# srv/pcl_feature_extraction

Hardware: AMD Instinct MI355X
Metric: Mpoints/s through NARF keypoint + FPFH descriptor on 1M-pt cloud (higher is better)
Workload: dtype f32; 1 GPU; configs[2] 1M-pt synthetic room, NARF(support 0.2) + normals(r 0.05) + FPFH(r 0.08) at the keypoints; image=640x480, parallelism=scan-per-gpu x1, descriptor_rows=83

## Files before the change

### pcl_feature_extraction_amd/csrc/pfx_grid.hip

```cpp
#include <algorithm>
#include <cstdlib>
#include <cstring>
#include <rocprim/rocprim.hpp>

#include "pfx_internal.h"

namespace pfx {
namespace {

__device__ __forceinline__ uint32_t f2ord(float f) {
  uint32_t u = __float_as_uint(f);
  return (u & 0x80000000u) ? ~u : (u | 0x80000000u);
}
__host__ __device__ __forceinline__ float ord2f(uint32_t u) {
  uint32_t b = (u & 0x80000000u) ? (u & 0x7fffffffu) : ~u;
  float f;
  memcpy(&f, &b, 4);
  return f;
}

constexpr int kBboxBlocks = 1024;
__global__ void __launch_bounds__(256) k_bbox(const float* __restrict__ x, const float* __restrict__ y,
                                              const float* __restrict__ z, int64_t n,
                                              uint32_t* __restrict__ mm) {
// ... 38 lines not shown
  uint32_t r[6] = {0xffffffffu, 0xffffffffu, 0xffffffffu, 0u, 0u, 0u};
  for (int b = t; b < nblocks; b += 256)
#pragma unroll
    for (int d = 0; d < 3; ++d) {
      r[d] = min(r[d], mm[b * 6 + d]);
      r[3 + d] = max(r[3 + d], mm[b * 6 + 3 + d]);
    }
#pragma unroll
  for (int d = 0; d < 6; ++d) s[d][t] = r[d];
  __syncthreads();
  for (int o = 128; o > 0; o >>= 1) {
    if (t < o)
#pragma unroll
      for (int d = 0; d < 3; ++d) {
        s[d][t] = min(s[d][t], s[d][t + o]);
        s[3 + d][t] = max(s[3 + d][t], s[3 + d][t + o]);
      }
    __syncthreads();
  }
  if (t < 6) mm[nblocks * 6 + t] = s[t][0];
}

__device__ __forceinline__ uint64_t lanemask_lt64() {
  const int lane = threadIdx.x & 63;
  return lane == 0 ? 0ull : (~0ull >> (64 - lane));
}

struct CellMap {
  double inv, ox, oy, oz, hx, hy, hz;
  int32_t nx, ny, nz;
};

__device__ __forceinline__ uint32_t point_key(const CellMap& m, float px, float py, float pz,
                                              int* __restrict__ oob) {
  uint32_t key = (uint32_t)((int64_t)m.nx * m.ny * m.nz);
  if (isfinite(px) && isfinite(py) && isfinite(pz)) {
    if (oob && ((double)px < m.ox || (double)py < m.oy || (double)pz < m.oz || (double)px > m.hx ||
                (double)py > m.hy || (double)pz > m.hz))
      atomicAdd(oob, 1);
    int64_t ix = (int64_t)floor(((double)px - m.ox) * m.inv);
    int64_t iy = (int64_t)floor(((double)py - m.oy) * m.inv);
    int64_t iz = (int64_t)floor(((double)pz - m.oz) * m.inv);
    ix = ix < 0 ? 0 : (ix >= m.nx ? m.nx - 1 : ix);
    iy = iy < 0 ? 0 : (iy >= m.ny ? m.ny - 1 : iy);
    iz = iz < 0 ? 0 : (iz >= m.nz ? m.nz - 1 : iz);
    key = (uint32_t)((ix * m.ny + iy) * m.nz + iz);
  }
  return key;
}

__global__ void __launch_bounds__(256) k_cell_keys(const float* __restrict__ x, const float* __restrict__ y,
                                                   const float* __restrict__ z, int64_t n, CellMap m,
                                                   uint32_t* __restrict__ keys, uint32_t* __restrict__ vals,
                                                   int* __restrict__ oob) {
  int64_t i = blockIdx.x * (int64_t)blockDim.x + threadIdx.x;
  if (i >= n) return;
  keys[i] = point_key(m, x[i], y[i], z[i], oob);
  vals[i] = (uint32_t)i;
}


constexpr int kCountBlock = 256;
constexpr int64_t kGridCountMaxPoints = int64_t(1) << 18;
constexpr int kAggRounds = 4;

__global__ void __launch_bounds__(256) k_count_zero(int32_t* __restrict__ p, int64_t m, int* __restrict__ oob) {
  for (int64_t i = blockIdx.x * (int64_t)blockDim.x + threadIdx.x; i < m; i += (int64_t)gridDim.x * blockDim.x)
    p[i] = 0;
  if (blockIdx.x == 0 && threadIdx.x == 0) *oob = 0;
}

__global__ void __launch_bounds__(kCountBlock) k_count_keys(const float* __restrict__ x, const float* __restrict__ y,
                                                            const float* __restrict__ z, int64_t n, CellMap m,
                                                            uint32_t* __restrict__ keys, uint32_t* __restrict__ rank,
                                                            int32_t* __restrict__ counts, int* __restrict__ oob) {
  const int64_t i = blockIdx.x * (int64_t)kCountBlock + threadIdx.x;
  const int lane = threadIdx.x & 63, wv = threadIdx.x >> 6;
  const uint32_t C = (uint32_t)((int64_t)m.nx * m.ny * m.nz);
  const bool live = i < n;
  uint32_t key = C;
  if (live) key = point_key(m, x[i], y[i], z[i], oob);
  const bool fin = live && key != C;
  uint64_t todo = __ballot(fin);
  int leader = lane, offs = 0, cnt = 1;
  for (int it = 0; it < kAggRounds && todo; ++it) {
    const int l = __builtin_ctzll(todo);
    const uint32_t k = (uint32_t)__shfl((int)key, l);
    const uint64_t same = __ballot(fin && key == k);
    if (fin && key == k) {
      leader = l;
      offs = __popcll(same & lanemask_lt64());
      cnt = __popcll(same);
    }
    todo &= ~same;
  }
  int base = 0;
  if (fin && lane == leader) base = atomicAdd(&counts[key], cnt);
  base = __shfl(base, leader);
  uint32_t r = (uint32_t)(base + offs);
  __shared__ int s_nf[kCountBlock / 64];
  const bool nf = live && !fin;
  const uint64_t bm = __ballot(nf);
  if (lane == 0) s_nf[wv] = __popcll(bm);
  __syncthreads();
  if (nf) {
    int before = __popcll(bm & lanemask_lt64());
    for (int w = 0; w < wv; ++w) before += s_nf[w];
    r = (uint32_t)before;
  }
// ... 37 lines not shown
    const int64_t last = s0 + 255 < n ? s0 + 255 : n - 1;
    const uint32_t k0 = skeys[s0], k1 = skeys[last];
    int64_t w0 = s0, w1 = s0;
    if (k0 < C) {
      w0 = cell_start[k0];
      w1 = cell_start[(k1 < C ? k1 : C - 1) + 1];
      w0 = w0 > s0 - kGridFatCap ? w0 : s0 - kGridFatCap;
      w1 = w1 < s0 + 256 + kGridFatCap ? w1 : s0 + 256 + kGridFatCap;
    }
    s_win[0] = w0;
    s_win[1] = w1;
  }
  __syncthreads();
  const int64_t w0 = s_win[0], w1 = s_win[1];
  for (int64_t t = w0 + threadIdx.x; t < w1; t += 256) s_idx[t - w0] = __float_as_uint(scr[t].w);
  __syncthreads();
  if (s >= n) return;
  const uint32_t key = skeys[s];
  const float4 v = scr[s];
  const uint32_t idx = __float_as_uint(v.w);
  int64_t d = s;
  if (key < C) {
    const int32_t start = cell_start[key], end = cell_start[key + 1];
    if (end - start > kGridFatCap) {
      if (s == start) atomicOr(oob, kGridFatBit);
      return;
    }
    const uint32_t* cell = s_idx + (start - w0);
    const int m = end - start;
    int before = 0;
    for (int t = 0; t < m; ++t) before += cell[t] < idx ? 1 : 0;
    d = (int64_t)start + before;
  }
  perm[d] = (int32_t)idx;
  sx[d] = v.x;
  sy[d] = v.y;
  sz[d] = v.z;
  sp[d] = make_float4(v.x, v.y, v.z, 0.0f);
}

__global__ void __launch_bounds__(256) k_fill_i32(int32_t* __restrict__ p, int64_t m, int32_t v) {
  for (int64_t i = blockIdx.x * (int64_t)blockDim.x + threadIdx.x; i < m; i += (int64_t)gridDim.x * blockDim.x)
    p[i] = v;
}

__global__ void __launch_bounds__(256) k_mark_starts(const uint32_t* __restrict__ skeys, int64_t n,
                                                     int32_t* __restrict__ cell_start) {
  const int64_t i = blockIdx.x * (int64_t)blockDim.x + threadIdx.x;
  if (i >= n) return;
  const uint32_t k = skeys[i];
  if (i == 0 || skeys[i - 1] != k) cell_start[k] = (int32_t)i;
}

__global__ void __launch_bounds__(256) k_gather_sorted(const float* __restrict__ x, const float* __restrict__ y,
                                                       const float* __restrict__ z, int64_t n,
                                                       const uint32_t* __restrict__ perm,
                                                       float* __restrict__ sx, float* __restrict__ sy,
                                                       float* __restrict__ sz, float4* __restrict__ sp) {
  int64_t i = blockIdx.x * (int64_t)blockDim.x + threadIdx.x;
  if (i >= n) return;
  uint32_t p = perm[i];
  const float a = x[p], b = y[p], c = z[p];
  sx[i] = a;
  sy[i] = b;
  sz[i] = c;
  sp[i] = make_float4(a, b, c, 0.0f);
}

__global__ void __launch_bounds__(256) k_fat_cells(const int32_t* __restrict__ cell_start, int64_t ncells,
                                                   int* __restrict__ flag) {
  const int64_t c = blockIdx.x * (int64_t)blockDim.x + threadIdx.x;
  if (c < ncells && cell_start[c + 1] - cell_start[c] > kGridFatCap) *flag = 1;
}

}

static bool bbox_dev(pfx_ctx* ctx, Grid& g, const float* d_x, const float* d_y, const float* d_z, int64_t n,
                     double lo[3], double hi[3]) {
  hipStream_t st = ctx->stream;
  uint32_t* mm = g.b_minmax.as<uint32_t>(6 * (kBboxBlocks + 1));
  const int blocks = (int)std::min<int64_t>(std::max<int64_t>(ceil_div(n, 1024), 1), kBboxBlocks);
  {
    TimeScope ts(ctx, "grid_bbox");
    k_bbox<<<blocks, 256, 0, st>>>(d_x, d_y, d_z, n, mm);
    k_bbox_reduce<<<1, 256, 0, st>>>(mm, blocks);
    check_launch("k_bbox");
  }
  uint32_t* h = ctx->readback<uint32_t>();
  PFX_HIP(hipMemcpyAsync(h, mm + 6 * blocks, sizeof(uint32_t) * 6, hipMemcpyDeviceToHost, st));
  ctx->sync_spin(st);
  uint32_t r[6];
  for (int d = 0; d < 6; ++d) r[d] = h[d];
  const bool any = r[0] != 0xffffffffu && r[3] != 0u;
  for (int d = 0; d < 3; ++d) {
    lo[d] = any ? ord2f(r[d]) : 0.0;
    hi[d] = any ? ord2f(r[3 + d]) : 0.0;
  }
  return any;
}

void points_bbox(pfx_ctx* ctx, Grid& g, const float* d_x, const float* d_y, const float* d_z, int64_t n,
                 double lo[3], double hi[3]) {
  bbox_dev(ctx, g, d_x, d_y, d_z, n, lo, hi);
}

void build_grid(pfx_ctx* ctx, Grid& g, const float* d_x, const float* d_y, const float* d_z,
                int64_t n, double radius, bool use_hint, bool fork_gather) {
  PFX_CHECK(n >= 0 && n < (int64_t(1) << 31), "point count must be in [0, 2^31)");
  PFX_CHECK(radius > 0.0, "radius must be > 0");
  ctx->join_side(ctx->stream);
  if (&g == &ctx->grid_b) {
    ctx->prep_x = nullptr;
    ctx->prep_n = -1;
    ctx->prep_qx = nullptr;
    ctx->prep_nq = -1;
  }
  hipStream_t st = ctx->stream;
  ++g.gen;
  g.n = n;
  g.ux = d_x; g.uy = d_y; g.uz = d_z;
  double lo[3] = {0, 0, 0}, hi[3] = {0, 0, 0};
  g.oob = nullptr;
  g.hint_user |= use_hint;
  if (use_hint && g.have_hint && n > 0) {
    for (int d = 0; d < 3; ++d) {
      lo[d] = g.hint_lo[d];
      hi[d] = g.hint_hi[d];
    }
    g.oob = g.b_oob.as<int>(1);
  } else if (n > 0) {
    bbox_dev(ctx, g, d_x, d_y, d_z, n, lo, hi);
    for (int d = 0; d < 3; ++d) {
      const double m = 0.1 * (hi[d] - lo[d]) + 2.0 * radius;
      g.hint_lo[d] = lo[d] - m;
      g.hint_hi[d] = hi[d] + m;
    }
    g.have_hint = true;
  }
  double cell = radius * (1.0 + 1e-6);
  const double max_cells = double(1 << 26);
  int64_t dims[3];
  for (int it = 0; it < 64; ++it) {
    for (int d = 0; d < 3; ++d) dims[d] = (int64_t)std::floor((hi[d] - lo[d]) / cell) + 1;
    double total = double(dims[0]) * double(dims[1]) * double(dims[2]);
    if (total <= max_cells) break;
    cell *= std::cbrt(total / max_cells) * 1.01;
  }
  g.cell = (float)cell;
  g.inv = (float)(1.0 / cell);
  g.ox = (float)lo[0]; g.oy = (float)lo[1]; g.oz = (float)lo[2];
  g.nx = (int32_t)dims[0]; g.ny = (int32_t)dims[1]; g.nz = (int32_t)dims[2];
  g.ncells = dims[0] * dims[1] * dims[2];
  const double inv = 1.0 / cell;
  g.inv = (float)inv;
  const int64_t C = g.ncells;

  const CellMap cm{inv, lo[0], lo[1], lo[2], hi[0], hi[1], hi[2], g.nx, g.ny, g.nz};
  g.dinv = inv;
  g.dox = lo[0]; g.doy = lo[1]; g.doz = lo[2];
  g.perm = g.b_perm.as<int32_t>(n + 1);
  g.sx = g.b_sx.as<float>(n + 1);
  g.sy = g.b_sy.as<float>(n + 1);
  g.sz = g.b_sz.as<float>(n + 1);
  g.sp = g.b_sp.as<float4>(n + 1);
  uint32_t* keys = g.b_keys.as<uint32_t>(n + 1);
  uint32_t* keys2 = g.b_keys2.as<uint32_t>(n + 1);
  uint32_t* vals = g.b_vals.as<uint32_t>(n + 1);
  g.skeys = keys2;

  if (g.oob && g.fat_pending) {
    PFX_HIP(hipEventSynchronize(g.fat_ev));
    g.fat_pending = false;
    g.fat = *g.h_fat != 0;
  }
  const char* mode = std::getenv("PFX_GRID_BUILD");
  const bool want_count = mode && std::strcmp(mode, "count") == 0
                              ? true
                              : (mode && std::strcmp(mode, "sort") == 0 ? false : n <= kGridCountMaxPoints);
  g.counted = g.oob != nullptr && n > 0 && want_count && !g.fat;
  ++ctx->stats[g.counted ? "grid_count_builds" : "grid_sort_builds"];
  if (g.oob && !g.counted) ++ctx->stats["grid_hinted_sort_builds"];
  if (g.counted) {
    const int64_t blocks = ceil_div(n, kCountBlock);
    const int64_t m = C + 1 + blocks;
    size_t scan_bytes = 0;
    PFX_HIP(rocprim::exclusive_scan(nullptr, scan_bytes, (int32_t*)nullptr, (int32_t*)nullptr, int32_t(0), (size_t)m,
                                    rocprim::plus<int32_t>(), st));
    void* tmp = g.b_tmp.get(scan_bytes + 16);
    g.cell_start = g.b_start.as<int32_t>(m + 1);
    float4* scr = g.b_scr.as<float4>(n + 1);
    TimeScope ts(ctx, "grid_build");
    k_count_zero<<<(unsigned)std::min<int64_t>(ceil_div(m, 256), 2048), 256, 0, st>>>(g.cell_start, m, g.oob);
    k_count_keys<<<(unsigned)blocks, kCountBlock, 0, st>>>(d_x, d_y, d_z, n, cm, keys, vals, g.cell_start, g.oob);
    check_launch("k_count_keys");
    PFX_HIP(rocprim::exclusive_scan(tmp, scan_bytes, g.cell_start, g.cell_start, int32_t(0), (size_t)m,
                                    rocprim::plus<int32_t>(), st));
    k_count_scatter<<<(unsigned)blocks, kCountBlock, 0, st>>>(d_x, d_y, d_z, n, (uint32_t)C, keys, vals, g.cell_start,
                                                              scr, keys2);
    k_count_order<<<(unsigned)ceil_div(n, 256), 256, 0, st>>>(scr, keys2, n, (uint32_t)C, g.cell_start, g.perm, g.sx,
                                                              g.sy, g.sz, g.sp, g.oob);
    check_launch("k_count_order");
    return;
  }

  using SortCfg = rocprim::radix_sort_config<rocprim::default_config, rocprim::default_config,
                                             rocprim::default_config, 0>;
  int bits = 1;
  while ((int64_t(1) << bits) <= C) ++bits;
  size_t sort_bytes = 0, scan_bytes = 0;
  PFX_HIP(rocprim::radix_sort_pairs<SortCfg>(nullptr, sort_bytes, (uint32_t*)nullptr, (uint32_t*)nullptr,
                                    (uint32_t*)nullptr, (uint32_t*)nullptr, (size_t)std::max<int64_t>(n, 1),
                                    0, bits, st));
  auto rev = rocprim::make_reverse_iterator(static_cast<int32_t*>(nullptr));
  PFX_HIP(rocprim::inclusive_scan(nullptr, scan_bytes, rev, rev, (size_t)(C + 1), rocprim::minimum<int32_t>(), st));
  void* tmp = g.b_tmp.get(std::max(sort_bytes, scan_bytes) + 16);
  g.cell_start = g.b_start.as<int32_t>(C + 2);
  {
    TimeScope ts(ctx, "grid_build");
    k_fill_i32<<<(unsigned)std::min<int64_t>(ceil_div(C + 2, 256), 2048), 256, 0, st>>>(g.cell_start, C + 2,
                                                                                       (int32_t)n);
    if (g.oob) k_fill_i32<<<1, 64, 0, st>>>(g.oob, 1, 0);
    if (n > 0) {
      k_cell_keys<<<(unsigned)ceil_div(n, 256), 256, 0, st>>>(d_x, d_y, d_z, n, cm, keys, vals, g.oob);
      check_launch("k_cell_keys");
      PFX_HIP(rocprim::radix_sort_pairs<SortCfg>(tmp, sort_bytes, keys, keys2, vals,
                                        reinterpret_cast<uint32_t*>(g.perm), (size_t)n, 0, bits, st));
      const bool forked = fork_gather && g.oob != nullptr;
      if (forked) ctx->fork_side(st);
      const auto gather = [&](hipStream_t s) {
        k_gather_sorted<<<(unsigned)ceil_div(n, 256), 256, 0, s>>>(d_x, d_y, d_z, n, reinterpret_cast<uint32_t*>(g.perm),
                                                                   g.sx, g.sy, g.sz, g.sp);
        check_launch("k_gather_sorted");
      };
      if (forked) gather(ctx->side);
      k_mark_starts<<<(unsigned)ceil_div(n, 256), 256, 0, st>>>(keys2, n, g.cell_start);
      auto r = rocprim::make_reverse_iterator(g.cell_start + C + 1);
      PFX_HIP(rocprim::inclusive_scan(tmp, scan_bytes, r, r, (size_t)(C + 1), rocprim::minimum<int32_t>(), st));
      if (!forked) gather(st);
    }
  }
  if (!g.oob && n > 0 && g.hint_user) {
    int* d_fat = g.b_fat.as<int>(1);
    if (!g.h_fat) PFX_HIP(hipHostMalloc((void**)&g.h_fat, 64, hipHostMallocDefault));
    if (!g.fat_ev) PFX_HIP(hipEventCreateWithFlags(&g.fat_ev, hipEventDisableTiming));
    if (g.fat_pending) PFX_HIP(hipEventSynchronize(g.fat_ev));
    k_fill_i32<<<1, 64, 0, st>>>(d_fat, 1, 0);
    k_fat_cells<<<(unsigned)ceil_div(C, 256), 256, 0, st>>>(g.cell_start, C, d_fat);
    check_launch("k_fat_cells");
    PFX_HIP(hipMemcpyAsync(g.h_fat, d_fat, sizeof(int), hipMemcpyDeviceToHost, st));
    PFX_HIP(hipEventRecord(g.fat_ev, st));
    g.fat_pending = true;
  }
}

}
```

### pcl_feature_extraction_amd/csrc/pfx_internal.h

```cpp
#pragma once
#include <hip/hip_runtime.h>
#include <stdint.h>
#include <cstdlib>

#include <map>
#include <stdexcept>
#include <string>
#include <vector>

#include "../../include/pfx.h"

namespace pfx {

struct Error : std::runtime_error {
  pfx_status code;
  Error(pfx_status c, const std::string& m) : std::runtime_error(m), code(c) {}
};

#define PFX_HIP(expr)                                                                   \
  do {                                                                                  \
    hipError_t _e = (expr);                                                             \
    if (_e != hipSuccess)                                                               \
      throw ::pfx::Error(PFX_ERR_DEVICE, std::string(#expr) + ": " + hipGetErrorString(_e)); \
  } while (0)

#define PFX_CHECK(cond, msg)                                                \
  do {                                                                      \
    if (!(cond)) throw ::pfx::Error(PFX_ERR_INVALID, std::string(msg));     \
  } while (0)

struct DevBuf {
  void* ptr = nullptr;
  size_t bytes = 0;
  void* get(size_t need) {
    if (need > bytes) {
      if (ptr) PFX_HIP(hipFree(ptr));
      size_t nb = need + need / 4 + 256;
      PFX_HIP(hipMalloc(&ptr, nb));
      bytes = nb;
    }
    return ptr;
  }
  template <class T> T* as(size_t count) { return static_cast<T*>(get(count * sizeof(T))); }
  void release() { if (ptr) (void)hipFree(ptr); ptr = nullptr; bytes = 0; }
};

struct KernelTimer {
  struct Pending { hipEvent_t a, b; std::string name; };
  bool enabled = false;
  bool stages_only = false;
  std::vector<Pending> pending;
  std::vector<hipEvent_t> pool;
  std::map<std::string, std::pair<double, int64_t> > acc;
  hipEvent_t take() {
    if (!pool.empty()) { hipEvent_t e = pool.back(); pool.pop_back(); return e; }
    hipEvent_t e;
    PFX_HIP(hipEventCreate(&e));
    return e;
  }
};

struct Grid {
  int64_t n = 0;
  float cell = 0.f, inv = 0.f, ox = 0.f, oy = 0.f, oz = 0.f;
  double dinv = 0.0, dox = 0.0, doy = 0.0, doz = 0.0;
  int32_t nx = 0, ny = 0, nz = 0;
  int64_t ncells = 0;
  float *sx = nullptr, *sy = nullptr, *sz = nullptr;
  float4* sp = nullptr;
  const float *ux = nullptr, *uy = nullptr, *uz = nullptr;
  int32_t* perm = nullptr;
  int32_t* cell_start = nullptr;
  const uint32_t* skeys = nullptr;
  DevBuf b_sx, b_sy, b_sz, b_sp, b_perm, b_start, b_keys, b_keys2, b_vals, b_tmp, b_minmax, b_oob, b_scr, b_fat;
  bool have_hint = false;
  double hint_lo[3] = {0, 0, 0}, hint_hi[3] = {0, 0, 0};
  int* oob = nullptr;
  mutable bool fat = false;
  int* h_fat = nullptr;
  hipEvent_t fat_ev = nullptr;
  bool fat_pending = false;
  bool hint_user = false;
  bool counted = false;
  uint64_t gen = 0;
  void release() {
    b_sx.release(); b_sy.release(); b_sz.release(); b_sp.release(); b_perm.release(); b_start.release();
    b_keys.release(); b_keys2.release(); b_vals.release(); b_tmp.release(); b_minmax.release(); b_oob.release();
    b_scr.release(); b_fat.release();
    if (fat_ev) { (void)hipEventSynchronize(fat_ev); (void)hipEventDestroy(fat_ev); fat_ev = nullptr; }
    if (h_fat) { (void)hipHostFree(h_fat); h_fat = nullptr; }
    fat_pending = false;
    have_hint = false;
    fat = false;
    oob = nullptr;
    ++gen;
  }
};

constexpr int kGridFatCap = 1024;
constexpr int kGridFatBit = 1 << 30;

struct GridView {
  const float *sx, *sy, *sz;
  const float4* sp;
  const float *ux, *uy, *uz;
  const int32_t* perm;
  const int32_t* cell_start;
  double inv, ox, oy, oz;
  int32_t nx, ny, nz;
};

enum ReportSlot {
  kRepFpfh, kRepPfh, kRepSpin, kRepIgrad, kRepRift, kRepSc, kRepLrf, kRepMoments, kRepPcurv, kReportSlots
};
constexpr int kReportWords = 16;
struct Reports {
  int* host = nullptr;
  bool pending[kReportSlots] = {};
  bool any() const {
    for (bool p : pending)
      if (p) return true;
    return false;
  }
};

struct NarfState;
struct NormalsState;
struct KeypointState;
struct IcpState;

}

struct pfx_ctx {
  int device = 0;
  hipStream_t own_stream = nullptr;
  hipStream_t stream = nullptr;
  bool on_own_stream = true;
  std::string last_error;
  bool shared_device = false;
  pfx::KernelTimer timer;
  std::map<std::string, int64_t> stats;
  pfx::Grid grid_a, grid_b;
  const float* prep_x = nullptr;
  int64_t prep_n = -1;
  double prep_r = 0.0;
  const float* prep_qx = nullptr;
  int64_t prep_nq = -1;
// ... 42 lines not shown
    PFX_HIP(hipEventRecord(fork_ev[1], side));
    PFX_HIP(hipStreamWaitEvent(st, fork_ev[1], 0));
  }
  void* host_rb = nullptr;
  template <class T> T* readback() {
    if (!host_rb) PFX_HIP(hipHostMalloc(&host_rb, 4096, hipHostMallocDefault));
    return static_cast<T*>(host_rb);
  }
  void* host_scratch = nullptr;
  size_t host_scratch_bytes = 0;
  void* pinned(size_t need) {
    if (need > host_scratch_bytes) {
      if (host_scratch) {
        PFX_HIP(hipStreamSynchronize(stream));
        PFX_HIP(hipHostFree(host_scratch));
      }
      host_scratch_bytes = need + need / 2 + 4096;
      PFX_HIP(hipHostMalloc(&host_scratch, host_scratch_bytes, hipHostMallocDefault));
    }
    return host_scratch;
  }
};

namespace pfx {

struct TimeScope {
  pfx_ctx* ctx;
  hipEvent_t a = nullptr, b = nullptr;
  std::string name;
  TimeScope(pfx_ctx* c, std::string n, bool stage = false) : ctx(c), name(std::move(n)) {
    if (ctx->timer.enabled && (stage || !ctx->timer.stages_only)) {
      a = ctx->timer.take();
      b = ctx->timer.take();
      PFX_HIP(hipEventRecord(a, ctx->stream));
    }
  }
  ~TimeScope() {
    if (a) {
      (void)hipEventRecord(b, ctx->stream);
      ctx->timer.pending.push_back(KernelTimer::Pending{a, b, name});
    }
  }
};

inline void check_launch(const char* what) {
  hipError_t e = hipGetLastError();
  if (e != hipSuccess)
    throw Error(PFX_ERR_DEVICE, std::string("launch ") + what + ": " + hipGetErrorString(e));
}

inline int64_t ceil_div(int64_t a, int64_t b) { return (a + b - 1) / b; }

void build_grid(pfx_ctx* ctx, Grid& g, const float* d_x, const float* d_y, const float* d_z,
                int64_t n, double radius, bool use_hint = false, bool fork_gather = false);
void points_bbox(pfx_ctx* ctx, Grid& g, const float* d_x, const float* d_y, const float* d_z, int64_t n,
                 double lo[3], double hi[3]);
inline void note_grid_word(pfx_ctx* ctx, const Grid& g, int word) {
  if (!(word & kGridFatBit)) return;
  g.fat = true;
  ++ctx->stats["grid_fat_fallbacks"];
}
inline GridView view(const Grid& g) {
  GridView v;
  v.sx = g.sx; v.sy = g.sy; v.sz = g.sz; v.sp = g.sp; v.perm = g.perm; v.cell_start = g.cell_start;
  v.ux = g.ux; v.uy = g.uy; v.uz = g.uz;
  v.inv = g.dinv; v.ox = g.dox; v.oy = g.doy; v.oz = g.doz; v.nx = g.nx; v.ny = g.ny; v.nz = g.nz;
  return v;
}

void normals_dev(pfx_ctx* ctx, const float* x, const float* y, const float* z, int64_t n,
                 double r, const float vp[3], float* nx, float* ny, float* nz, float* curv);
void normals_lists_dev(pfx_ctx* ctx, const float* x, const float* y, const float* z, int64_t n, double r,
                       float* nx, float* ny, float* nz, float* curv);
void normals_chains_dev(pfx_ctx* ctx, pfx_ctx* owner, const uint8_t* mask, int want, const float vp[3], float* nx,
                        float* ny, float* nz, float* curv);
void normals_release(pfx_ctx* ctx);
void normals_grid_launch_dev(pfx_ctx* ctx, const float* x, const float* y, const float* z, int64_t n, double r);
void normals_launch_dev(pfx_ctx* ctx, const float* x, const float* y, const float* z, int64_t n, double r,
                        const float vp[3], float* nx, float* ny, float* nz, float* curv);
bool normals_finish_dev(pfx_ctx* ctx);
void normals_prepare_dev(pfx_ctx* ctx, const float* x, const float* y, const float* z, int64_t n, double r);
void normals_subset_dev(pfx_ctx* ctx, const float* x, const float* y, const float* z, int64_t n, double r,
                        const uint8_t* mask, int want, const float vp[3], float* nx, float* ny, float* nz,
                        float* curv);
void normals_fast_dev(pfx_ctx* ctx, const float* x, const float* y, const float* z, int64_t n, double r,
                      const float vp[3], float* nx, float* ny, float* nz, float* curv);
double cloud_resolution_dev(pfx_ctx* ctx, const float* x, const float* y, const float* z, int64_t n);
int64_t iss_keypoints_dev(pfx_ctx* ctx, const float* x, const float* y, const float* z, int64_t n, double salient,
                          double non_max, int min_nb, double g21, double g32, int32_t* out, int64_t cap,
                          double* third_out);
void keypoints_release(pfx_ctx* ctx);
struct IcpResult {
  float T[16];
  double fitness;
  int converged, iterations, state;
};
void icp_dev(pfx_ctx* ctx, const float* sx, const float* sy, const float* sz, int64_t ns, const float* tx,
             const float* ty, const float* tz, int64_t nt, const pfx_icp_params& p, const float* guess,
             IcpResult& out, float* ax, float* ay, float* az);
void icp_release(pfx_ctx* ctx);
int64_t ransac_rejector(pfx_ctx* ctx, const float* sx, const float* sy, const float* sz, int64_t ns,
                        const float* tx, const float* ty, const float* tz, int64_t nt, const int32_t* query,
                        const int32_t* match, int64_t n, double threshold, int max_iterations, int32_t* keep_out,
                        float* T_out, int64_t* iters_out);
int64_t harris3d_dev(pfx_ctx* ctx, const float* x, const float* y, const float* z, int64_t n, double radius,
                     float threshold, int refine, int32_t* out, int64_t cap, float* resp_out, float* corners_out,
                     int64_t* n_corners, int32_t* corner_idx_out = nullptr);
// ... 87 lines not shown
```

### pcl_feature_extraction_amd/csrc/pfx_nblist.h

```cpp
#pragma once
#include "pfx_internal.h"
#include "pfx_neighbors.h"

namespace pfx {

constexpr uint32_t kEntryOffMask = 0x0fffffffu;
__host__ __device__ __forceinline__ int entry_run(uint32_t e) { return (int)(e >> 28); }
__host__ __device__ __forceinline__ uint32_t entry_off(uint32_t e) { return e & kEntryOffMask; }
constexpr uint8_t kLgCompact = 0x80;

__host__ __device__ __forceinline__ uint32_t widen_entry16(uint32_t e16) {
  return ((e16 >> 12) << 28) | (e16 & 0xfffu);
}
constexpr int kLaneMaxCompact = 2048;
__device__ __forceinline__ uint32_t list_entry(const uint32_t* list, int64_t off, int lgr, int m) {
  const int64_t i = off + ((int64_t)m << (lgr & 0x7f));
  return (lgr & kLgCompact) ? widen_entry16(reinterpret_cast<const uint16_t*>(list)[i]) : list[i];
}

struct NbLists {
  int64_t nq = 0;
  int64_t total = 0;
  int64_t long_total = 0;
  int64_t long_nq = 0;
// ... 14 lines not shown
constexpr int kLaneListLanes = 256;
constexpr int kLaneListTable = 9 * kLaneListLanes;

struct LaneList {
  int32_t p;
  int k;
  const uint32_t* lst;
  int lg;
  const int32_t* s_rt;
  int tid;

  __device__ __forceinline__ LaneList(const GridView& g, const NbLists& L, int64_t j, int32_t* table)
      : p(L.qpos[j]), s_rt(table), tid(threadIdx.x) {
    const uint32_t key = L.skeys[p];
#pragma unroll
    for (int r = 0; r < 9; ++r) {
      int32_t s, len;
      block_run(g, key, r, s, len);
      table[r * kLaneListLanes + tid] = s;
    }
    lst = L.list + L.off[j];
    lg = L.lg[j];
    k = L.cnt[j];
  }
  __device__ __forceinline__ uint32_t entry(int m) const { return lst[(int64_t)m << lg]; }
  __device__ __forceinline__ int32_t pos(int m) const {
    const uint32_t e = entry(m);
    return s_rt[entry_run(e) * kLaneListLanes + tid] + (int32_t)entry_off(e);
  }
  __device__ __forceinline__ int32_t idx(const GridView& g, int m) const { return g.perm[pos(m)]; }
};

constexpr int kLongList = 1024;

struct NormalsState {
  NbLists L;
  int64_t n = 0;
  const float *x = nullptr, *y = nullptr, *z = nullptr;
  double r = 0.0;
  bool ready = false;
  uint64_t grid_gen = 0;
  bool pending = false;
  bool nlong_zeroed = false;
  uint64_t grid_ahead_gen = 0;
  const float *grid_ahead_x = nullptr, *grid_ahead_y = nullptr, *grid_ahead_z = nullptr;
  int64_t grid_ahead_n = 0;
  double grid_ahead_r = 0.0;
  float vp[3] = {0.f, 0.f, 0.f};
  float *nx = nullptr, *ny = nullptr, *nz = nullptr, *curv = nullptr;
};

void build_lists(pfx_ctx* ctx, const Grid& g, const uint8_t* mask, double radius, bool sorted, NbLists& out,
                 const char* tag, bool defer = false, int want = 1, bool compact = false, bool gate = false);
bool build_lists_check(pfx_ctx* ctx, const Grid& g, NbLists& out, const char* tag);

}
```

### pcl_feature_extraction_amd/csrc/pfx_nblist.hip

```cpp
#include <cstdlib>
#include <cstring>
#include <rocprim/rocprim.hpp>

#include "pfx_nblist.h"
#include "pfx_neighbors.h"

namespace pfx {
namespace {

constexpr int kQ = 16;
typedef float pf2 __attribute__((ext_vector_type(2)));
constexpr int kArena = 16384;
constexpr int kArenaQuery = 16384;
constexpr int kTcapSmall = 384, kTcapSparse = 1280, kTcapDense = 8000;
constexpr int kCapQuery = 4096, kBucketsQuery = 1024;
constexpr int kCapMid8 = 8192, kBucketsMid8 = 1024;
constexpr int kCapMid = 16384, kBucketsMid = 2048;
#ifndef PFX_HUGE_BLOCKS
#define PFX_HUGE_BLOCKS 1024
#endif
constexpr int kCapHuge = 1 << 18, kBucketsHuge = 4096, kHugeBlocks = PFX_HUGE_BLOCKS;
#ifndef PFX_NT_QUERY
#define PFX_NT_QUERY 512
#endif
// ... 1572 lines not shown
  ListBuild(pfx_ctx* c, const Grid& grid, const char* t, double radius, bool sorted, bool compact_)
      : ctx(c), G(grid), tag(t), st(c->stream), n(grid.n), g(view(grid)), rr((float)(radius * radius)),
        isort(sorted ? 1 : 0), compact(compact_ ? 1 : 0), lb(buf("list")), hs(buf("scratch")) {
    qpos = buf("qpos").as<int32_t>(n);
    d_nq = buf("nq").as<int64_t>(1);
    flags = buf("flags").as<uint8_t>(n);
    seg = buf("seg").as<int32_t>(n);
    tiles = buf("tiles").as<int32_t>(n);
    d_ntiles = buf("ntiles").as<int64_t>(1);
    recs = buf("recs").as<int32_t>((size_t)2 * n * kRecInts);
    q4k = buf("single").as<int32_t>(n);
    qhuge = buf("huge").as<int32_t>(n);
    off = buf("off").as<int64_t>(n);
    cnt = buf("cnt").as<int32_t>(n);
    lgs = buf("lg").as<uint8_t>(n);
    counters = buf("counters").as<int>(kNCounters);
    wq = buf("wide").as<int32_t>((size_t)n);
    q16k = buf("mid").as<int32_t>(n);
    q8k = buf("mid8").as<int32_t>(n);
    qrec = buf("qrec").as<int32_t>((size_t)n * kRecInts);
    cursor = buf("cursor").as<unsigned long long>(4);
    PFX_HIP(rocprim::select(nullptr, t1, rocprim::counting_iterator<int32_t>(0), flags, qpos, d_nq, (size_t)n, st));
    PFX_HIP(rocprim::inclusive_scan(nullptr, t2, seg, seg, (size_t)n, rocprim::maximum<int32_t>(), st));
    PFX_HIP(rocprim::select(nullptr, t3, rocprim::counting_iterator<int32_t>(0), flags, tiles, d_ntiles, (size_t)n,
                            st));
    tmp = buf("tmp").get(std::max(t1, std::max(t2, t3)) + 16);
    tq_dev = static_cast<TierQ*>(buf("tierq").get(sizeof(TierQ)));
    if (!lb.ptr) {
      size_t words = 64 * (size_t)(n + 1);
      if (const char* e = std::getenv("PFX_LIST_WORDS")) words = std::max<size_t>(256, std::strtoull(e, nullptr, 10));
      lb.get(sizeof(uint32_t) * words);
    }
    const int heavy = (int)std::min<int64_t>(4, n >> 21);
    ch_small = 4;
    ch_sparse = std::max(2, heavy);
    ch_dense = std::max(1, heavy);
  }

  size_t list_words() const { return lb.bytes / sizeof(uint32_t); }
  ListOut list_out() const {
    return ListOut{off, cnt, lgs, static_cast<uint32_t*>(lb.ptr), cursor, list_words(), compact, qrec};
  }

  void setup(const uint8_t* mask, int want) {
    const unsigned nb = (unsigned)ceil_div(n, 256);
    const TierQ tq{{q4k, q8k, q16k, qhuge},
                   {counters + kWork4k, counters + kWork8k, counters + kWork16k, counters + kWorkHuge}};
    TimeScope ts(ctx, std::string(tag) + "_tiles");
    if (mask) {
      k_list_init<<<1, 256, 0, st>>>(nullptr, 0, nullptr, d_nq, counters, kNCounters, cursor, tq, tq_dev);
      k_mask_flags<<<nb, 256, 0, st>>>(G.perm, G.skeys, n, (uint64_t)G.ncells, mask, want, flags);
      PFX_HIP(rocprim::select(tmp, t1, rocprim::counting_iterator<int32_t>(0), flags, qpos, d_nq, (size_t)n, st));
    } else {
      k_list_init<<<nb, 256, 0, st>>>(qpos, n, G.cell_start + G.ncells, d_nq, counters, kNCounters, cursor, tq,
                                      tq_dev);
      const char* mode = std::getenv("PFX_LIST_SETUP");
      const bool cells = !(mode && std::strcmp(mode, "scan") == 0);
      ++ctx->stats[std::string(tag) + (cells ? "_setup_cells" : "_setup_scan")];
      if (cells) {
        k_tile_cells<<<(unsigned)ceil_div(n, kSlice), 256, 0, st>>>(g, G.skeys, G.ncells, recs, n, wq, counters);
        check_launch("nblist cell tiles");
        return;
      }
    }
    k_seg_marks<<<nb, 256, 0, st>>>(qpos, G.skeys, d_nq, seg);
    PFX_HIP(rocprim::inclusive_scan(tmp, t2, seg, seg, (size_t)n, rocprim::maximum<int32_t>(), st));
    k_tile_flags<<<nb, 256, 0, st>>>(seg, d_nq, flags, n);
    PFX_HIP(rocprim::select(tmp, t3, rocprim::counting_iterator<int32_t>(0), flags, tiles, d_ntiles, (size_t)n, st));
    k_tile_class<<<nb, 256, 0, st>>>(g, qpos, G.skeys, d_nq, tiles, d_ntiles, recs, n, wq, counters);
    check_launch("nblist tiles");
  }

  void reset_for_retry() {
    PFX_HIP(hipMemsetAsync(cursor, 0, 4 * sizeof(unsigned long long), st));
    PFX_HIP(hipMemsetAsync(counters + kRetryFirst, 0, (kNCounters - kRetryFirst) * sizeof(int), st));
  }

  template <int CAP, int NB, bool GLOBAL, int NT, int WPE>
  void launch_tier(unsigned grid, const int32_t* work, Counter count, Counter head, uint32_t* scratch,
                   const char* what) {
    const auto kern = k_nb_query<CAP, NB, GLOBAL, NT, WPE>;
    const size_t lds = GLOBAL ? 0 : sizeof(uint32_t) * 2 * CAP;
    if (lds) PFX_HIP(hipFuncSetAttribute((const void*)kern, hipFuncAttributeMaxDynamicSharedMemorySize, (int)lds));
    kern<<<grid, NT, lds, st>>>(g, work, counters + count, rr, (float)NB / rr, isort, list_out(),
                                GLOBAL ? nullptr : tq_dev, counters + kOverCap, scratch, counters + head);
    check_launch(what);
  }
  void launch_4k() {
    launch_tier<kCapQuery, kBucketsQuery, false, kNtQuery, PFX_Q_WPE>(kGrid4k, q4k, kWork4k, kHead4k, nullptr,
                                                                      "nblist 4k lists");
  }
  void launch_8k() {
    launch_tier<kCapMid8, kBucketsMid8, false, kNtMid8, kNtMid8 / 128>(kGrid8k, q8k, kWork8k, kHead8k, nullptr,
                                                                        "nblist 8k lists");
  }
  void launch_16k() {
    launch_tier<kCapMid, kBucketsMid, false, kNtMid, kNtMid / 256>(kGrid16k, q16k, kWork16k, kHead16k, nullptr,
                                                                    "nblist 16k lists");
  }
  unsigned huge_blocks() const { return (unsigned)std::min<size_t>(kGridHugeMax, hs.bytes / kHugeSlice); }
  void launch_huge() {
    launch_tier<kCapHuge, kBucketsHuge, true, kNtHuge, 4>(huge_blocks(), qhuge, kWorkHuge, kHeadHuge,
                                                          static_cast<uint32_t*>(hs.ptr), "nblist huge lists");
  }

  void launch_lists(int ran) {
    const ListOut lo = list_out();
    const float bscale = 256.0f / rr;
// ... 28 lines not shown
      TimeScope ts_query(ctx, std::string(tag) + "_lists_query");
      launch_4k();
      if (ran & kRan8k) launch_8k();
      if (ran & kRan16k) launch_16k();
      if (hs.ptr) launch_huge();
    }
    check_launch("nblist lists");
  }

  void defer_to_check(int ran, NbLists& out) {
    int64_t* d_nq_eff = buf("nq_eff").as<int64_t>(1);
    k_defer_gate<<<1, 64, 0, st>>>(counters, cursor, list_words(), hs.ptr ? 1 : 0, ran, G.oob, d_nq, d_nq_eff);
    check_launch("k_defer_gate");
    point(out);
    out.nq = n;
    out.nq_dev = d_nq_eff;
  }

  const ListsRb* read_back() { return pfx::read_back(ctx, counters, cursor, d_nq, nullptr); }
  int lack(const ListsRb* rb, int ran) const {
    return lists_lack(rb->cnt, rb->cur[0], list_words(), hs.ptr != nullptr, ran, rb->oob);
  }

  void catch_up(int lacking, int ran) {
    auto rewind = [&](Counter head, Counter count) {
      PFX_HIP(hipMemcpyAsync(counters + head, counters + count, sizeof(int), hipMemcpyDeviceToDevice, st));
    };
    if (ran & kRan16k) rewind(kHead16k, kWork16k);
    if (hs.ptr) rewind(kHeadHuge, kWorkHuge);
    if (lacking & kRan8k) launch_8k();
    launch_16k();
    if (hs.ptr) launch_huge();
  }

  void huge_alloc(int count) { hs.get(kHugeSlice * (size_t)std::min(kGridHugeMax, std::max(kCUs, count))); }

  void regrow(unsigned long long demand) {
    lb.release();
    lb.get(sizeof(uint32_t) * ((size_t)demand + kArenaTails + ((size_t)1 << 20)));
  }

  void point(NbLists& out) const {
    out.qpos = qpos;
    out.off = off;
    out.cnt = cnt;
    out.lg = lgs;
    out.list = static_cast<const uint32_t*>(lb.ptr);
    out.compact = compact != 0;
    out.list_cap = (int64_t)list_words();
    out.skeys = G.skeys;
  }
};

}

bool build_lists_check(pfx_ctx* ctx, const Grid& G, NbLists& out, const char* tag) {
  auto B = [&](const char* what) -> DevBuf& { return ctx->bufs[bname(tag, what)]; };
  const ListsRb* rb = read_back(ctx, B("counters").ptr, B("cursor").ptr, B("nq").ptr, G.oob);
  note_grid_word(ctx, G, rb->oob);
  const size_t words = B("list").bytes / sizeof(uint32_t);
  const int ran = (int)ctx->stats[std::string(tag) + "_ran_mid_tiers"];
  const int lacking = lists_lack(rb->cnt, rb->cur[0], words, B("scratch").ptr != nullptr, ran, rb->oob);
  if (lacking & (kLackGrid | kLackBuffer | kLackScratch)) return false;
  note_mid_tiers(ctx, tag, rb->cnt);
  if (lacking) return false;
  if (rb->cnt[kOverCap] > 0) throw_over_cap(tag, rb->cnt[kOverCap]);
  publish(ctx, tag, *rb, words, out);
  return true;
}

void build_lists(pfx_ctx* ctx, const Grid& G, const uint8_t* mask, double radius, bool sorted, NbLists& out,
                 const char* tag, bool defer, int want, bool compact, bool gate) {
  out = NbLists();
  if (G.n == 0) return;
  if (G.n >= (int64_t(1) << 28))
    throw Error(PFX_ERR_CAPACITY, std::string(tag) + ": neighbour lists support < 2^28 points");
  ListBuild b(ctx, G, tag, radius, sorted, compact);
  b.setup(mask, want);
  ctx->join_side(b.st);
  if (gate && ctx->lists_gate) {
    PFX_HIP(hipStreamWaitEvent(b.st, ctx->lists_gate, 0));
    ctx->lists_gate = nullptr;
  }
  for (int attempt = 0; attempt < 3; ++attempt) {
    if (attempt) b.reset_for_retry();
    int ran = attempt ? kRanAll : wanted_tiers(ctx, tag);
    ctx->stats[std::string(tag) + "_ran_mid_tiers"] = ran;
    b.launch_lists(ran);
    if (defer && attempt == 0) {
      b.defer_to_check(ran, out);
      return;
    }
    const ListsRb* rb = b.read_back();
    int lacking = b.lack(rb, ran);
    if (lacking & kRanWide) {
      note_mid_tiers(ctx, tag, rb->cnt);
      ++ctx->stats[std::string(tag) + "_wide_reruns"];
      continue;
    }
    if (lacking & (kRan8k | kRan16k)) {
      b.catch_up(lacking, ran);
      ran = kRanAll;
      rb = b.read_back();
      lacking = b.lack(rb, ran);
      ++ctx->stats[std::string(tag) + "_tier_catchups"];
    }
// ... 28 lines not shown
```

### pcl_feature_extraction_amd/csrc/pfx_normals.hip

```cpp
#include <cstring>
#include <algorithm>
#include <cstdio>
#include <cstdlib>
#include <mutex>

#include <rocprim/rocprim.hpp>

#include "pfx_nblist.h"
#include "pfx_neighbors.h"
#include "pfx_normal_math.h"

namespace pfx {
namespace {

constexpr int kBatch = 8;
#ifndef PFX_LANE_MAX
#define PFX_LANE_MAX (2 * kLongList)
#endif
constexpr int kLaneMax = PFX_LANE_MAX;
static_assert(kLaneMax >= kLaneMaxCompact, "lists up to kLaneMaxCompact must take the lane-per-query chains");

#ifndef PFX_LANE_DENSE_MUL
#define PFX_LANE_DENSE_MUL 2
#endif
// ... 705 lines not shown
    PFX_HIP(hipStreamSynchronize(st));
    ctx->stats["normals_long_lists"] = h[0];
    ctx->stats["normals_chain_wg_staged"] = h[1];
    ctx->stats["normals_chain_wg_table"] = h[2];
    ctx->stats["normals_chain_wg_lane"] = h[3];
    ctx->stats["normals_chain_wg_deferred"] = h[4];
  }
#ifdef PFX_SHOT_PROFILE
  {
    unsigned long long pr[16];
    PFX_HIP(hipStreamSynchronize(st));
    PFX_HIP(hipMemcpyFromSymbol(pr, HIP_SYMBOL(g_chain_prof), sizeof(pr)));
    for (int b = 0; b < 16; b += 8)
      fprintf(stderr, "chain%s: WGs %llu prologue %.0f cyc/WG | waves %llu chain %.0f cyc/wave, max k %.1f/wave, "
              "%.1f cyc/step, mean k %.1f/lane\n", b ? "_big" : "", pr[b + 4], pr[b + 0] / (double)(pr[b + 4] + !pr[b + 4]), pr[b + 3],
              pr[b + 1] / (double)(pr[b + 3] + !pr[b + 3]), pr[b + 2] / (double)(pr[b + 3] + !pr[b + 3]),
              pr[b + 1] / (double)(pr[b + 2] + !pr[b + 2]), pr[b + 5] / 64.0 / (double)(pr[b + 3] + !pr[b + 3]));
    const unsigned long long z[16] = {};
    PFX_HIP(hipMemcpyToSymbol(HIP_SYMBOL(g_chain_prof), z, sizeof(z)));
  }
#endif
}

namespace {

bool normals_speculative_lists(pfx_ctx* ctx, const float* x, const float* y, const float* z, int64_t n, double r,
                               float* nx, float* ny, float* nz, float* curv) {
  if (n == 0) return false;
  if (!ctx->normals) ctx->normals = new NormalsState();
  NormalsState& ns = *ctx->normals;
  ns.ready = false;
  ns.pending = false;
  ns.n = n;
  ns.x = x;
  ns.y = y;
  ns.z = z;
  ns.r = r;
  ns.L = NbLists();
  TimeScope phase(ctx, "normals_lists_phase", true);
  const bool ahead = ns.grid_ahead_gen != 0 && ns.grid_ahead_gen == ctx->grid_a.gen && ns.grid_ahead_x == x &&
                     ns.grid_ahead_y == y && ns.grid_ahead_z == z && ns.grid_ahead_n == n && ns.grid_ahead_r == r;
  ns.grid_ahead_gen = 0;
  struct SideJoin {
    pfx_ctx* ctx;
    ~SideJoin() {
      try {
        ctx->join_side(ctx->stream);
      } catch (...) {
      }
    }
  } side_join{ctx};
  const char* fork_env = std::getenv("PFX_GATHER_FORK");
  const bool fork_gather = !(fork_env && std::strcmp(fork_env, "0") == 0);
  if (!ahead) build_grid(ctx, ctx->grid_a, x, y, z, n, r, true, fork_gather);
  ctx->stats["normals_gather_forked"] += ctx->side_pending ? 1 : 0;
  int* n_long = ctx->buf("normals_nlong").as<int>(kNLong);
  k_nan_fill4<<<(unsigned)std::min<int64_t>(ceil_div(n, 256), 4096), 256, 0,
                ctx->side_pending ? ctx->side : ctx->stream>>>(nx, ny, nz, curv, n, n_long, kNLong);
  check_launch("k_nan_fill4");
  ns.nlong_zeroed = true;
  build_lists(ctx, ctx->grid_a, nullptr, r, true, ns.L, "normals", true, 1, true,
              true);
  return true;
}

bool normals_conclude(pfx_ctx* ctx, bool ok, const float* x, const float* y, const float* z, int64_t n, double r,
                      const float vp[3], float* nx, float* ny, float* nz, float* curv) {
  NormalsState& ns = *ctx->normals;
  ctx->grid_a.oob = nullptr;
  ctx->stats["normals_speculative_reruns"] += ok ? 0 : 1;
  if (ok) {
    ctx->stats["normals_neighbors"] = ns.L.total;
    ctx->stats["normals_long_neighbors"] = ns.L.long_total;
    ctx->stats["normals_long_queries"] = ns.L.long_nq;
    ctx->stats["normals_queries"] = ns.L.nq;
    ctx->normals_fork_hint = ns.L.long_nq * 8 <= ns.L.nq;
    return true;
  }
  normals_lists_dev(ctx, x, y, z, n, r, nx, ny, nz, curv);
  normals_chains_dev(ctx, ctx, nullptr, 0, vp, nx, ny, nz, curv);
  return false;
}
}

void normals_dev(pfx_ctx* ctx, const float* x, const float* y, const float* z, int64_t n, double r,
                 const float vp[3], float* nx, float* ny, float* nz, float* curv) {
  GateScope gate_scope(ctx);
  TimeScope total(ctx, "normals", true);
  PFX_CHECK(r > 0.0, "normals: radius must be > 0");
  PFX_CHECK(n >= 0, "normals: negative point count");
  if (normals_speculative_lists(ctx, x, y, z, n, r, nx, ny, nz, curv)) {
    NormalsState& ns = *ctx->normals;
    const bool ok = build_lists_check(ctx, ctx->grid_a, ns.L, "normals");
    ns.ready = true;
    if (ok) normals_chains_dev(ctx, ctx, nullptr, 0, vp, nx, ny, nz, curv);
    normals_conclude(ctx, ok, x, y, z, n, r, vp, nx, ny, nz, curv);
    return;
  }
  normals_lists_dev(ctx, x, y, z, n, r, nx, ny, nz, curv);
  if (n > 0) normals_chains_dev(ctx, ctx, nullptr, 0, vp, nx, ny, nz, curv);
}

void normals_launch_dev(pfx_ctx* ctx, const float* x, const float* y, const float* z, int64_t n, double r,
                        const float vp[3], float* nx, float* ny, float* nz, float* curv) {
  GateScope gate_scope(ctx);
  TimeScope total(ctx, "normals", true);
  PFX_CHECK(r > 0.0, "normals: radius must be > 0");
// ... 91 lines not shown
```

Baseline: 219.4 Mpoints/s.

## Replace fill+mark+min-scan cell starts with one fused kernel folding list init

Builds the grid's cell_start array in a single kernel. Slice blocks write each run boundary directly, and stripe blocks binary-search the sorted keys to fill the gaps between runs. This replaces the full-array fill, the mark-starts kernel and the reverse min-scan. The same kernel also performs the neighbor-list init work (qpos iota, counter and cursor reset, tier-queue blob copy), and the OOB word is double-buffered and zeroed inside k_cell_keys, which removes several small launches. The cost is considerably more complex code with packed 16-bit fields and extra coupling between grid build and list setup.

```diff
diff --git a/pcl_feature_extraction_amd/csrc/pfx_grid.hip b/pcl_feature_extraction_amd/csrc/pfx_grid.hip
--- a/pcl_feature_extraction_amd/csrc/pfx_grid.hip
+++ b/pcl_feature_extraction_amd/csrc/pfx_grid.hip
@@ -114,9 +114,10 @@
 __global__ void __launch_bounds__(256) k_cell_keys(const float* __restrict__ x, const float* __restrict__ y,
                                                    const float* __restrict__ z, int64_t n, CellMap m,
                                                    uint32_t* __restrict__ keys, uint32_t* __restrict__ vals,
-                                                   int* __restrict__ oob) {
+                                                   int* __restrict__ oob, int* __restrict__ oob_other) {
   int64_t i = blockIdx.x * (int64_t)blockDim.x + threadIdx.x;
   if (i >= n) return;
+  if (i == 0 && oob_other) *oob_other = 0;
   keys[i] = point_key(m, x[i], y[i], z[i], oob);
   vals[i] = (uint32_t)i;
 }
@@ -260,6 +261,101 @@
   if (i == 0 || skeys[i - 1] != k) cell_start[k] = (int32_t)i;
 }
 
+constexpr int kStartsSlice = 4096;
+constexpr int kStartsStripeBits = 11;
+__global__ void __launch_bounds__(256) k_cell_starts(const uint32_t* __restrict__ skeys, int64_t n, int64_t C,
+                                                     int32_t* __restrict__ cell_start, int nslices, GridTail tail) {
+  constexpr int slice = kStartsSlice;
+  constexpr int64_t T = int64_t(1) << kStartsStripeBits;
+  const int tid = threadIdx.x;
+  if ((int)blockIdx.x >= nslices) {
+    const int64_t S = (int64_t)(blockIdx.x - nslices) << kStartsStripeBits;
+    const int64_t E = S + T < C + 2 ? S + T : C + 2;
+    int64_t lo = 0, hi = n;
+    while (hi > lo) {
+      const int64_t step = (hi - lo + 255) / 256;
+      const int64_t at = lo + tid * step;
+      const int below = __syncthreads_count(at < hi && (int64_t)skeys[at] < E);
+      if (below == 0) {
+        hi = lo;
+      } else {
+        const int64_t h = lo + below * step;
+        lo = lo + (below - 1) * step + 1;
+        hi = h < hi ? h : hi;
+      }
+    }
+    const int64_t p = lo;
+    const int64_t k = p < n ? (int64_t)skeys[p] : C + 1;
+    const int64_t kp = p > 0 ? (int64_t)skeys[p - 1] : -1;
+    const int64_t c0 = kp + 1 > S ? kp + 1 : S;
+    const int64_t c1 = k - T < E - 1 ? k - T : E - 1;
+    for (int64_t c = c0 + tid; c <= c1; c += 256) cell_start[c] = (int32_t)p;
+    return;
+  }
+  __shared__ uint32_t s_key[kStartsSlice + 2];
+  __shared__ int32_t s_first[kStartsSlice + 1];
+  __shared__ uint32_t s_what[kStartsSlice + 1];
+  __shared__ int s_qn;
+  static_assert(kStartsStripeBits <= 16 && kStartsSlice <= 4096, "the packing of s_what");
+  const int64_t s0 = blockIdx.x * (int64_t)slice;
+  int m = (int)(n - s0 < slice ? n - s0 : slice);
+  {
+    uint32_t kr[kStartsSlice / 256];
+#pragma unroll
+    for (int i = 0; i < kStartsSlice / 256; ++i) kr[i] = tid + 256 * i < m ? skeys[s0 + tid + 256 * i] : 0u;
+#pragma unroll
+    for (int i = 0; i < kStartsSlice / 256; ++i)
+      if (tid + 256 * i < m) s_key[1 + tid + 256 * i] = kr[i];
+  }
+  if (tid == 0) {
+    s_key[0] = s0 > 0 ? skeys[s0 - 1] : 0xffffffffu;
+    s_qn = 0;
+    if (s0 + m == n) s_key[1 + m] = (uint32_t)(C + 1);
+  }
+  if (tail.qpos) {
+    for (int t = tid; t < m; t += 256) tail.qpos[s0 + t] = (int32_t)(s0 + t);
+    if (blockIdx.x == 0) {
+      if (tid < tail.ncounters) tail.counters[tid] = 0;
+      if (tid < 4) tail.cursor[tid] = 0ull;
+      if (tid == 0) {
+#pragma unroll
+        for (int w = 0; w < 8; ++w) tail.blob_dst[w] = tail.blob[w];
+      }
+    }
+  }
+  if (s0 + m == n) ++m;
+  __syncthreads();
+  for (int t = tid; t < m; t += 256) {
+    if (s_key[1 + t] == s_key[t]) continue;
+    const int64_t k = (int64_t)s_key[1 + t];
+    const int64_t kp = (s0 == 0 && t == 0) ? -1 : (int64_t)s_key[t];
+    const int64_t first = kp + 1 > k - (T - 1) ? kp + 1 : k - (T - 1);
+    if (tail.d_nq && k >= C && kp < C) *tail.d_nq = s0 + t;
+    if (k - first < 2) {
+      for (int64_t c = first; c <= k; ++c) cell_start[c] = (int32_t)(s0 + t);
+    } else {
+      const int e = atomicAdd(&s_qn, 1);
+      s_first[e] = (int32_t)first;
+      s_what[e] = ((uint32_t)t << 16) | (uint32_t)(k - first);
+    }
+  }
+  __syncthreads();
+  const int qn = s_qn, lane = tid & 63, wv = tid >> 6;
+  for (int base = 64 * wv; base < qn; base += 256) {
+    const int mine = base + lane < qn ? base + lane : qn - 1;
+    const int32_t f_l = s_first[mine];
+    const uint32_t w_l = s_what[mine];
+    const int ne = qn - base < 64 ? qn - base : 64;
+    for (int j = 0; j < ne; ++j) {
+      const int32_t f = __builtin_amdgcn_readlane(f_l, j);
+      const uint32_t w = (uint32_t)__builtin_amdgcn_readlane((int)w_l, j);
+      const int last = (int)(w & 0xffffu);
+      const int32_t v = (int32_t)(s0 + (w >> 16));
+      for (int c = lane; c <= last; c += 64) cell_start[(int64_t)f + c] = v;
+    }
+  }
+}
+
 __global__ void __launch_bounds__(256) k_gather_sorted(const float* __restrict__ x, const float* __restrict__ y,
                                                        const float* __restrict__ z, int64_t n,
                                                        const uint32_t* __restrict__ perm,
@@ -313,7 +409,7 @@
 }
 
 void build_grid(pfx_ctx* ctx, Grid& g, const float* d_x, const float* d_y, const float* d_z,
-                int64_t n, double radius, bool use_hint, bool fork_gather) {
+                int64_t n, double radius, bool use_hint, bool fork_gather, const GridTail* tail) {
   PFX_CHECK(n >= 0 && n < (int64_t(1) << 31), "point count must be in [0, 2^31)");
   PFX_CHECK(radius > 0.0, "radius must be > 0");
   ctx->join_side(ctx->stream);
@@ -325,6 +421,7 @@
   }
   hipStream_t st = ctx->stream;
   ++g.gen;
+  g.folded_init = nullptr;
   g.n = n;
   g.ux = d_x; g.uy = d_y; g.uz = d_z;
   double lo[3] = {0, 0, 0}, hi[3] = {0, 0, 0};
@@ -335,7 +432,13 @@
       lo[d] = g.hint_lo[d];
       hi[d] = g.hint_hi[d];
     }
-    g.oob = g.b_oob.as<int>(1);
+    const bool fresh = g.b_oob.ptr == nullptr;
+    int* words = g.b_oob.as<int>(2);
+    if (fresh) {
+      PFX_HIP(hipMemsetAsync(words, 0, 2 * sizeof(int), ctx->stream));
+      g.oob_next = 0;
+    }
+    g.oob = words + g.oob_next;
   } else if (n > 0) {
     bbox_dev(ctx, g, d_x, d_y, d_z, n, lo, hi);
     for (int d = 0; d < 3; ++d) {
@@ -388,6 +491,16 @@
   g.counted = g.oob != nullptr && n > 0 && want_count && !g.fat;
   ++ctx->stats[g.counted ? "grid_count_builds" : "grid_sort_builds"];
   if (g.oob && !g.counted) ++ctx->stats["grid_hinted_sort_builds"];
+  int* oob_other = nullptr;
+  if (g.oob) {
+    int* words = g.oob - g.oob_next;
+    if (g.counted) {
+      g.oob = words + (1 - g.oob_next);
+    } else {
+      oob_other = words + (1 - g.oob_next);
+      g.oob_next = 1 - g.oob_next;
+    }
+  }
   if (g.counted) {
     const int64_t blocks = ceil_div(n, kCountBlock);
     const int64_t m = C + 1 + blocks;
@@ -425,11 +538,15 @@
   g.cell_start = g.b_start.as<int32_t>(C + 2);
   {
     TimeScope ts(ctx, "grid_build");
-    k_fill_i32<<<(unsigned)std::min<int64_t>(ceil_div(C + 2, 256), 2048), 256, 0, st>>>(g.cell_start, C + 2,
-                                                                                       (int32_t)n);
-    if (g.oob) k_fill_i32<<<1, 64, 0, st>>>(g.oob, 1, 0);
+    const char* starts_env = std::getenv("PFX_CELL_STARTS");
+    const bool scan_starts = n == 0 || (starts_env && std::strcmp(starts_env, "scan") == 0);
+    ctx->stats["grid_starts_scan"] += scan_starts ? 1 : 0;
+    ctx->stats["grid_starts_fill"] += scan_starts ? 0 : 1;
+    if (scan_starts)
+      k_fill_i32<<<(unsigned)std::min<int64_t>(ceil_div(C + 2, 256), 2048), 256, 0, st>>>(g.cell_start, C + 2,
+                                                                                         (int32_t)n);
     if (n > 0) {
-      k_cell_keys<<<(unsigned)ceil_div(n, 256), 256, 0, st>>>(d_x, d_y, d_z, n, cm, keys, vals, g.oob);
+      k_cell_keys<<<(unsigned)ceil_div(n, 256), 256, 0, st>>>(d_x, d_y, d_z, n, cm, keys, vals, g.oob, oob_other);
       check_launch("k_cell_keys");
       PFX_HIP(rocprim::radix_sort_pairs<SortCfg>(tmp, sort_bytes, keys, keys2, vals,
                                         reinterpret_cast<uint32_t*>(g.perm), (size_t)n, 0, bits, st));
@@ -441,9 +558,19 @@
         check_launch("k_gather_sorted");
       };
       if (forked) gather(ctx->side);
-      k_mark_starts<<<(unsigned)ceil_div(n, 256), 256, 0, st>>>(keys2, n, g.cell_start);
-      auto r = rocprim::make_reverse_iterator(g.cell_start + C + 1);
-      PFX_HIP(rocprim::inclusive_scan(tmp, scan_bytes, r, r, (size_t)(C + 1), rocprim::minimum<int32_t>(), st));
+      if (scan_starts) {
+        k_mark_starts<<<(unsigned)ceil_div(n, 256), 256, 0, st>>>(keys2, n, g.cell_start);
+        auto r = rocprim::make_reverse_iterator(g.cell_start + C + 1);
+        PFX_HIP(rocprim::inclusive_scan(tmp, scan_bytes, r, r, (size_t)(C + 1), rocprim::minimum<int32_t>(), st));
+      } else {
+        const int nslices = (int)ceil_div(n, kStartsSlice);
+        const int nstripes = (int)ceil_div(C + 2, int64_t(1) << kStartsStripeBits);
+        const bool fold = tail && tail->qpos && g.oob != nullptr;
+        k_cell_starts<<<(unsigned)(nslices + nstripes), 256, 0, st>>>(keys2, n, C, g.cell_start, nslices,
+                                                                      fold ? *tail : GridTail());
+        if (fold) g.folded_init = tail->qpos;
+        check_launch("k_cell_starts");
+      }
       if (!forked) gather(st);
     }
   }
diff --git a/pcl_feature_extraction_amd/csrc/pfx_internal.h b/pcl_feature_extraction_amd/csrc/pfx_internal.h
--- a/pcl_feature_extraction_amd/csrc/pfx_internal.h
+++ b/pcl_feature_extraction_amd/csrc/pfx_internal.h
@@ -58,6 +58,16 @@
     PFX_HIP(hipEventCreate(&e));
     return e;
   }
+};
+
+struct GridTail {
+  int32_t* qpos = nullptr;
+  int64_t* d_nq = nullptr;
+  int* counters = nullptr;
+  int ncounters = 0;
+  unsigned long long* cursor = nullptr;
+  uint64_t blob[8] = {};
+  uint64_t* blob_dst = nullptr;
 };
 
 struct Grid {
@@ -76,6 +86,7 @@
   bool have_hint = false;
   double hint_lo[3] = {0, 0, 0}, hint_hi[3] = {0, 0, 0};
   int* oob = nullptr;
+  int oob_next = 0;
   mutable bool fat = false;
   int* h_fat = nullptr;
   hipEvent_t fat_ev = nullptr;
@@ -83,6 +94,7 @@
   bool hint_user = false;
   bool counted = false;
   uint64_t gen = 0;
+  mutable const void* folded_init = nullptr;
   void release() {
     b_sx.release(); b_sy.release(); b_sz.release(); b_sp.release(); b_perm.release(); b_start.release();
     b_keys.release(); b_keys2.release(); b_vals.release(); b_tmp.release(); b_minmax.release(); b_oob.release();
@@ -93,6 +105,7 @@
     have_hint = false;
     fat = false;
     oob = nullptr;
+    oob_next = 0;
     ++gen;
   }
 };
@@ -241,7 +254,8 @@
 inline int64_t ceil_div(int64_t a, int64_t b) { return (a + b - 1) / b; }
 
 void build_grid(pfx_ctx* ctx, Grid& g, const float* d_x, const float* d_y, const float* d_z,
-                int64_t n, double radius, bool use_hint = false, bool fork_gather = false);
+                int64_t n, double radius, bool use_hint = false, bool fork_gather = false,
+                const GridTail* tail = nullptr);
 void points_bbox(pfx_ctx* ctx, Grid& g, const float* d_x, const float* d_y, const float* d_z, int64_t n,
                  double lo[3], double hi[3]);
 inline void note_grid_word(pfx_ctx* ctx, const Grid& g, int word) {
diff --git a/pcl_feature_extraction_amd/csrc/pfx_nblist.h b/pcl_feature_extraction_amd/csrc/pfx_nblist.h
--- a/pcl_feature_extraction_amd/csrc/pfx_nblist.h
+++ b/pcl_feature_extraction_amd/csrc/pfx_nblist.h
@@ -90,6 +90,7 @@
 
 void build_lists(pfx_ctx* ctx, const Grid& g, const uint8_t* mask, double radius, bool sorted, NbLists& out,
                  const char* tag, bool defer = false, int want = 1, bool compact = false, bool gate = false);
+GridTail lists_init_tail(pfx_ctx* ctx, int64_t n, const char* tag);
 bool build_lists_check(pfx_ctx* ctx, const Grid& g, NbLists& out, const char* tag);
 
 }
diff --git a/pcl_feature_extraction_amd/csrc/pfx_nblist.hip b/pcl_feature_extraction_amd/csrc/pfx_nblist.hip
--- a/pcl_feature_extraction_amd/csrc/pfx_nblist.hip
+++ b/pcl_feature_extraction_amd/csrc/pfx_nblist.hip
@@ -1648,8 +1648,12 @@
       k_mask_flags<<<nb, 256, 0, st>>>(G.perm, G.skeys, n, (uint64_t)G.ncells, mask, want, flags);
       PFX_HIP(rocprim::select(tmp, t1, rocprim::counting_iterator<int32_t>(0), flags, qpos, d_nq, (size_t)n, st));
     } else {
-      k_list_init<<<nb, 256, 0, st>>>(qpos, n, G.cell_start + G.ncells, d_nq, counters, kNCounters, cursor, tq,
-                                      tq_dev);
+      const bool folded = G.folded_init == qpos;
+      G.folded_init = nullptr;
+      ctx->stats[std::string(tag) + "_init_folded"] += folded ? 1 : 0;
+      if (!folded)
+        k_list_init<<<nb, 256, 0, st>>>(qpos, n, G.cell_start + G.ncells, d_nq, counters, kNCounters, cursor, tq,
+                                        tq_dev);
       const char* mode = std::getenv("PFX_LIST_SETUP");
       const bool cells = !(mode && std::strcmp(mode, "scan") == 0);
       ++ctx->stats[std::string(tag) + (cells ? "_setup_cells" : "_setup_scan")];
@@ -1784,6 +1788,25 @@
   }
 };
 
+}
+
+GridTail lists_init_tail(pfx_ctx* ctx, int64_t n, const char* tag) {
+  GridTail t;
+  const char* mode = std::getenv("PFX_LIST_SETUP");
+  if (n <= 0 || n >= (int64_t(1) << 28) || (mode && std::strcmp(mode, "scan") == 0)) return t;
+  auto B = [&](const char* what) -> DevBuf& { return ctx->bufs[bname(tag, what)]; };
+  t.qpos = B("qpos").as<int32_t>(n);
+  t.d_nq = B("nq").as<int64_t>(1);
+  t.counters = B("counters").as<int>(kNCounters);
+  t.ncounters = kNCounters;
+  t.cursor = B("cursor").as<unsigned long long>(4);
+  int* c = t.counters;
+  const TierQ tq{{B("single").as<int32_t>(n), B("mid8").as<int32_t>(n), B("mid").as<int32_t>(n), B("huge").as<int32_t>(n)},
+                 {c + kWork4k, c + kWork8k, c + kWork16k, c + kWorkHuge}};
+  static_assert(sizeof(TierQ) == sizeof(t.blob), "GridTail::blob holds a TierQ");
+  std::memcpy(t.blob, &tq, sizeof(tq));
+  t.blob_dst = static_cast<uint64_t*>(B("tierq").get(sizeof(TierQ)));
+  return t;
 }
 
 bool build_lists_check(pfx_ctx* ctx, const Grid& G, NbLists& out, const char* tag) {
diff --git a/pcl_feature_extraction_amd/csrc/pfx_normals.hip b/pcl_feature_extraction_amd/csrc/pfx_normals.hip
--- a/pcl_feature_extraction_amd/csrc/pfx_normals.hip
+++ b/pcl_feature_extraction_amd/csrc/pfx_normals.hip
@@ -781,7 +781,10 @@
   } side_join{ctx};
   const char* fork_env = std::getenv("PFX_GATHER_FORK");
   const bool fork_gather = !(fork_env && std::strcmp(fork_env, "0") == 0);
-  if (!ahead) build_grid(ctx, ctx->grid_a, x, y, z, n, r, true, fork_gather);
+  if (!ahead) {
+    const GridTail tail = lists_init_tail(ctx, n, "normals");
+    build_grid(ctx, ctx->grid_a, x, y, z, n, r, true, fork_gather, &tail);
+  }
   ctx->stats["normals_gather_forked"] += ctx->side_pending ? 1 : 0;
   int* n_long = ctx->buf("normals_nlong").as<int>(kNLong);
   k_nan_fill4<<<(unsigned)std::min<int64_t>(ceil_div(n, 256), 4096), 256, 0,
```

Measured after the change: 221.4 Mpoints/s (median of 6 runs). About the same (+0.9%).
